# ssteinberg/wave_tracer

Measured on AMD Instinct MI355X. Metric: Msamples/sec (whole node), cornell-box 1440^2 wave-mode, higher is better.
Workload: dtype f32

## Files before the change

### wave_tracer_amd/api.py

```python
import ctypes as C
import json
import math
import os

_HERE = os.path.dirname(os.path.abspath(__file__))

os.environ.setdefault("HSA_KERNARG_POOL_SIZE", str(16 << 20))


def lib_path():
    return os.environ.get("WTGPU_LIB") or os.path.join(_HERE, "libwtgpu.so")


class WtgpuError(RuntimeError):
    pass


class SceneParams(C.Structure):
    _fields_ = [("res", C.c_uint32), ("max_depth", C.c_int32), ("fsd", C.c_int32), ("mis", C.c_int32), ("rr", C.c_int32),
                ("force_ray_tracing", C.c_int32), ("mesh_detail", C.c_int32), ("lut_n_theta", C.c_uint32), ("lut_m", C.c_uint32),
                ("polarimetric", C.c_int32)]


class TestHooks(C.Structure):
# ... 65 lines not shown


SYMBOLS = ["wtgpu_scene_create_named", "wtgpu_scene_create_from_desc", "wtgpu_scene_get_info", "wtgpu_scene_host_desc",
           "wtgpu_scene_upload", "wtgpu_render", "wtgpu_trace_rays", "wtgpu_traverse_cones", "wtgpu_get_counters",
           "wtgpu_reset_counters", "wtgpu_last_render_timings", "wtgpu_develop", "wtgpu_scene_destroy", "wtgpu_last_error",
           "wtgpu_scene_stats_json", "wtgpu_calibrate_copy", "wtgpu_render_async", "wtgpu_join", "wtgpu_query_regions", "wtgpu_render_progressive",
           "wtgpu_cancel", "wtgpu_pause", "wtgpu_resume", "wtgpu_capture_intermediate", "wtgpu_comm_unique_id", "wtgpu_comm_create", "wtgpu_film_reduce", "wtgpu_comm_destroy", "wtgpu_scene_create_from_xml",
           "wtgpu_scene_shape_id", "wtgpu_scene_sensor_mask_spec", "wtgpu_sensor_mask", "wtgpu_sensor_mask_host",
           "wtgpu_scene_tonemap_spec", "wtgpu_develop_device", "wtgpu_tonemap_device", "wtgpu_tonemap_host",
           "wtgpu_film_stats_edges", "wtgpu_film_stats_device", "wtgpu_film_stats_host",
           "wtgpu_film_compare_device", "wtgpu_film_compare_host"]
PROGRESS_CB = C.CFUNCTYPE(C.c_int, C.c_uint64, C.c_uint64, C.c_void_p)
CAPTURE_CB = C.CFUNCTYPE(None, C.c_uint64, C.c_void_p)

_lib = None


def load_library():
    global _lib
    if _lib is not None:
        return _lib
    p = lib_path()
    if not os.path.exists(p):
        raise WtgpuError(f"{p} is missing: build it with `python -c 'import __graft_entry__ as g; g.build()'` "
                         f"(hipcc --offload-arch=gfx950); wave_tracer_amd has no CPU fallback")
    os.environ.setdefault("HSA_KERNARG_POOL_SIZE", str(16 << 20))
    try:
        import torch
    except ImportError:
        pass
# ... 541 lines not shown
        def call(spec, rec, planes):
            if diff:
                d["diff"] = np.zeros((self.height, self.width, planes), dtype=np.float32)
            _check(load_library().wtgpu_film_compare_host(self._h, *(t.ctypes.data for t in sets[0]), int(spe_a), *(t.ctypes.data for t in sets[1]), int(spe_b),
                                                          C.byref(spec), None if m is None else m.ctypes.data, int(threads), C.cast(rec, C.c_void_p),
                                                          d["diff"].ctypes.data if diff else None))
        out = self._film_compare(call, stokes_component, abs, luminance, eps)
        out.update(d)
        return out

    def profile_counters(self, n=8):
        out = (C.c_uint64 * n)()
        _check(load_library().wtgpu_test_profile_counters(self._h, out, n))
        return [int(v) for v in out]

    def counters(self):
        c = Counters()
        _check(load_library().wtgpu_get_counters(self._h, C.byref(c)))
        return c.as_dict()

    def reset_counters(self):
        _check(load_library().wtgpu_reset_counters(self._h))

    def trace_ab_stats(self):
        a, b, d, w, r = C.c_double(0), C.c_double(0), C.c_uint64(0), C.c_uint64(0), C.c_uint64(0)
        _check(load_library().wtgpu_trace_ab_stats(self._h, C.byref(a), C.byref(b), C.byref(d), C.byref(w), C.byref(r)))
        return {"ms_refill": a.value, "ms_sm": b.value, "differing_words": int(d.value), "walks": int(w.value), "rounds": int(r.value)}

    def timings(self):
        t = (C.c_float * 12)()
# ... 46 lines not shown
```

### wave_tracer_amd/csrc/kernels_connect.hip

```cpp
#include "wtgpu_kernels.h"

namespace wtk {

WT_D bool strategy_valid(const integrator_opts_t& o, int s, int t, int nS, int nT) {
    const int depth = t + s - 2;
    if (t > nT || s > nS) return false;
    if ((t == 1 && s == 1) || depth < 0 || depth > o.max_depth) return false;
    if (!o.emitter_direct && s == 1) return false;
    if (!o.sensor_direct && t == 1) return false;
    if (o.debug_only_s && (int)o.debug_only_s - 1 != s) return false;
    if (o.debug_only_t && (int)o.debug_only_t - 1 != t) return false;
    return true;
}
WT_D bool strategy_class_valid(const integrator_opts_t& o, int sk, int tk, int nS, int nT) {
    const int K = (int)kKeyDim - 1;
    const int t1 = tk < K ? tk : nT, s1 = sk < K ? sk : nS;
    for (int t = tk; t <= t1; ++t)
        for (int s = sk; s <= s1; ++s)
            if (strategy_valid(o, s, t, nS, nT)) return true;
    return false;
}
WT_D int wave_max_i(int v) {
#pragma unroll
    for (int off = 32; off > 0; off >>= 1) v = max(v, __shfl_xor(v, off, 64));
    return v;
}

__global__ void __launch_bounds__(kEnumBlock) k_connect_enum(launch_args_t a) {
    __shared__ uint32_t s_cnt[kNumKeys], s_base[kNumKeys];
    const uint32_t i = blockIdx.x * kEnumBlock + threadIdx.x;
    const size_t W2 = 2 * (size_t)a.st.cap;
    for (uint32_t k = threadIdx.x; k < kNumKeys; k += kEnumBlock) s_cnt[k] = 0;
    int nT = -1, nS = -1;
    if (i < a.nb) {
        nT = (int)a.st.walks[(size_t)(i) * a.st.walk_words + WT_WALK_NVERTS_WORD];
        nS = (int)a.st.walks[(size_t)(a.st.cap + i) * a.st.walk_words + WT_WALK_NVERTS_WORD];
#pragma unroll
        for (int c = 0; c < 4; ++c) a.st.lacc[(size_t)c * a.st.cap + i] = 0.0;
    }
    __syncthreads();
    const int K = (int)kKeyDim - 1;
    const int kT = nT < K ? nT : K, kS = nS < K ? nS : K;
    for (int tk = 0; tk <= kT; ++tk)
        for (int sk = 0; sk <= kS; ++sk)
            if (strategy_class_valid(a.sc.opts, sk, tk, nS, nT)) atomicAdd(&s_cnt[(uint32_t)tk * kKeyDim + (uint32_t)sk], 1u);
    __syncthreads();
    for (uint32_t k = threadIdx.x; k < kNumKeys; k += kEnumBlock) {
        const uint32_t c = s_cnt[k];
        s_base[k] = c ? atomicAdd(a.st.strat_count + k, c) : 0u;
        s_cnt[k] = 0;
    }
    __syncthreads();
    for (int tk = 0; tk <= kT; ++tk)
        for (int sk = 0; sk <= kS; ++sk)
            if (strategy_class_valid(a.sc.opts, sk, tk, nS, nT)) {
                const uint32_t key = (uint32_t)tk * kKeyDim + (uint32_t)sk;
                a.st.strat_items[(size_t)key * a.st.cap + s_base[key] + atomicAdd(&s_cnt[key], 1u)] = i;
            }
}
__global__ void __launch_bounds__(64) k_connect_scan(launch_args_t a) {
    if (a.st.ext)
        for (uint32_t q = threadIdx.x; q < a.st.ext->n_chunks * kChunkCtlWords; q += 64) a.st.ext->chunk_ctl[q] = 0;
    if (threadIdx.x == 0) {
        uint32_t acc = 0;
        for (uint32_t k = 0; k < kNumKeys; ++k) {
            const uint32_t c = a.st.strat_count[k];
            a.st.strat_prefix[k] = acc;
            acc += c;
            a.st.strat_count[k] = 0;
        }
        a.st.strat_prefix[kNumKeys] = acc;
        a.st.ctl[CTL_STRAT_HEAD] = 0;
        a.st.ctl[CTL_STRAT_HEAD_OPEN] = 0;

    }
}
template <bool OPEN>
WT_D void connect_strat_body(const launch_args_t& a) {
    __shared__ stack_entry_t lds[kLdsStack * kBlock];
    __shared__ uint32_t s_prefix[kNumKeys + 1];
    constexpr int K = (int)kKeyDim - 1;
    if (!OPEN) {
        for (uint32_t k = threadIdx.x; k <= kNumKeys; k += kBlock) s_prefix[k] = a.st.strat_prefix[k];
    } else if (threadIdx.x == 0) {
        uint32_t acc = 0;
        for (uint32_t k = 0; k < kNumKeys; ++k) {
            s_prefix[k] = acc;
            if ((int)(k / kKeyDim) == K || (int)(k % kKeyDim) == K) acc += a.st.strat_prefix[k + 1] - a.st.strat_prefix[k];
        }
// ... 42 lines not shown
                one(sk, tk);
            } else {
                const int nT = (int)a.st.walks[(size_t)i * a.st.walk_words + WT_WALK_NVERTS_WORD];
                const int nS = (int)a.st.walks[((size_t)a.st.cap + i) * a.st.walk_words + WT_WALK_NVERTS_WORD];
                const int t1 = tk == K ? nT : tk, s1 = sk == K ? nS : sk;
                for (int t = tk; t <= t1; ++t)
                    for (int s = sk; s <= s1; ++s)
                        if (strategy_valid(a.sc.opts, s, t, nS, nT)) one(s, t);
            }
        }
    }
    if (a.count_stats) flush_counters(a.st.counters, ctr);
}
__global__ void __launch_bounds__(kBlock, WTGPU_LB_CONNECT) k_connect_strat(launch_args_t a) { connect_strat_body<false>(a); }
__global__ void __launch_bounds__(kBlock, WTGPU_LB_CONNECT) k_connect_strat_open(launch_args_t a) { connect_strat_body<true>(a); }
constexpr uint32_t kPendShadow = 0x80000000u;
WT_D void pending_append(const launch_args_t& a, uint32_t* cctl, bool keep, uint32_t i, int s, int t, const connect_ret_t& cr) {
    const bdpt_ext_t& x = *a.st.ext;
    const unsigned long long m = __ballot(keep);
    if (!m) return;
    const int lane = threadIdx.x & 63;
    const int leader = __ffsll((long long)m) - 1;
    uint32_t base = 0;
    if (lane == leader) base = atomicAdd(cctl + CHUNK_PEND_COUNT, (uint32_t)__popcll(m));
    base = (uint32_t)__shfl((int)base, leader, 64);
    const uint32_t slot = base + (uint32_t)__popcll(m & ((1ull << lane) - 1ull));
    if (!keep || slot >= x.pend_cap) return;
    conn_pending_t r;
    r.i = i;
    r.st = (uint32_t)s | ((uint32_t)t << 16) | (cr.need_shadow ? kPendShadow : 0u);
// ... 215 lines not shown
```

### wave_tracer_amd/csrc/wtgpu.hip

```cpp
#include "wtgpu_host.h"

thread_local std::string g_err;

static void note_rounds(wtgpu_scene* s, uint32_t n) { s->rounds_hist[s->rounds_hist_n++ % 8u] = n; }
static int drain_rec(wtgpu_scene* s, chunk_rec_t& r) {
    if (!r.busy) return WTGPU_OK;
    HIP_CHECK(hipEventSynchronize(r.ev[r.ev_final]));
    const uint32_t rounds = r.h_ctl[CTL_ROUNDS];
    s->cap_hits += r.h_ctl[CTL_COUNT0 + (r.rounds_launched & 1u)] + r.h_ctl[CTL_BACK0 + (r.rounds_launched & 1u)];
    s->acc[4] += rounds;
    s->acc[5] += rounds;
    s->acc[6] += 1;
    s->rounds_launched_total += r.rounds_launched;
    if (s->knobs.timing) {
        auto elapsed = [](hipEvent_t a, hipEvent_t b) {
            float ms = 0.f;
            return hipEventElapsedTime(&ms, a, b) == hipSuccess ? ms : 0.f;
        };
        s->acc[0] += elapsed(r.ev[0], r.ev[1]);
        size_t e = 1;
        for (uint32_t k = 0; k < r.rounds_timed; ++k, e += 6) {
            static const int slot[6] = {1, 7, 2, 8, 9, 10};
            for (int q = 0; q < 6; ++q) s->acc[slot[q]] += elapsed(r.ev[e + q], r.ev[e + q + 1]);
        }
// ... 144 lines not shown
            HP_LAUNCH(k_interact_c_hard, dim3(std::max<uint32_t>(1u, gh / K.grid_div_hard)), dim3(WTGPU_HARD_BLOCK), 0, st_, a, in);
            rec(r, st_);
        }
        r.rounds_launched = r_end;
        return WTGPU_OK;
    }
    void light(const launch_args_t& a, hipStream_t st_, uint32_t launched) {
        if (path_mode || !K.light_rounds || launched >= K.max_rounds) return;
        HP_LAUNCH(k_light_rounds, dim3(1), dim3(kBlock), 0, st_, a, (int)(launched & 1u), launched, K.max_rounds - launched);
    }
    int tail(const launch_args_t& a, chunk_rec_t& r, hipStream_t st_) {
        const uint32_t nb = a.nb, gf = g_full(nb);
        if (path_mode) {
            HP_LAUNCH(k_path_flush, dim3(kFlushGrid), dim3(kBlock), 0, st_, a, (int)(r.rounds_launched & 1u));
        } else {
            HP_LAUNCH(k_connect_enum, dim3((nb + kEnumBlock - 1) / kEnumBlock), dim3(kEnumBlock), 0, st_, a);
            HP_LAUNCH(k_connect_scan, dim3(1), dim3(64), 0, st_, a);
            const bool open = (uint32_t)s->host.opts.max_depth + 2 >= kKeyDim - 1;
            if (K.staged_connect && !open) {
                for (uint32_t c = 0; c < s->n_chunks; ++c) {
                    const uint32_t g = c == 0 ? gf : std::max<uint32_t>(1u, gf / 8u);
                    HP_LAUNCH(k_connect_eval, dim3(g), dim3(kBlock), 0, st_, a, c);
                    HP_LAUNCH(k_connect_shadow, dim3(g), dim3(kBlock), 0, st_, a, c);
                    HP_LAUNCH(k_connect_mis, dim3(g), dim3(kBlock), 0, st_, a, c);
                }
            } else {
                HP_LAUNCH(k_connect_strat, dim3(gf), dim3(kBlock), 0, st_, a);
                if (open) HP_LAUNCH(k_connect_strat_open, dim3(std::max<uint32_t>(1u, gf / 8u)), dim3(kBlock), 0, st_, a);
            }
            const uint32_t fw = a.film.width, fh = a.film.height, planes = film_planes(s->host.sensor);
            if (K.tiled_splat && s->host.sensor.rf_radius <= 1 && planes <= 16 && (uint64_t)nb * 2u >= (uint64_t)a.npix)
                HP_LAUNCH(k_connect_splat_tiled, dim3(fh * ((fw + kBlock - 1) / kBlock)), dim3(kBlock), 3 * kSplatCols * (planes + 1) * sizeof(double), st_, a);
            else
                HP_LAUNCH(k_connect_splat, dim3((nb + kBlock - 1) / kBlock), dim3(kBlock), 0, st_, a);
        }
        HIP_CHECK(hipGetLastError());
        HIP_CHECK(hipMemcpyAsync(r.h_ctl, a.st.ctl, CTL_WORDS * sizeof(uint32_t), hipMemcpyDeviceToHost, st_));
        r.ev_final = s->knobs.timing ? r.ev_used : 0;
        HIP_CHECK(hipEventRecord(r.ev[r.ev_final], st_));
        if (ev_fail) return fail(WTGPU_ERR_HIP, "hipEventRecord failed");
// ... 229 lines not shown
```

### wave_tracer_amd/csrc/wtgpu_kernels.h

```cpp
#pragma once
#include <hip/hip_runtime.h>

#include <cstddef>
#include <cstdint>
#include <cstring>

#include "../../include/wtgpu.h"
#include "wt/bdpt.h"
#include "wt/coop.h"
#include "wt/coop_fsd.h"
#include "wt/coop_utd.h"
#include "wt/path.h"

using namespace wt;
namespace wt {
struct tonemap_args_t;
}

namespace wtk {


#ifndef WTGPU_LB_TRACE
#define WTGPU_LB_TRACE 3
#endif
// ... 23 lines not shown
constexpr int kLdsStack = WTGPU_LDS_STACK;
constexpr uint32_t kConeBudget = 96;
constexpr int kSpillStack = 64 - kLdsStack;

enum : uint32_t { CTL_STRAT_HEAD_OPEN = 25, CTL_UTD_COUNT0 = 26, CTL_UTD_COUNT1 = 27, CTL_FSDQ_COUNT0 = 28, CTL_FSDQ_COUNT1 = 29, CTL_FSDQ_HEAD = 30, CTL_NEEQ_COUNT = 31, CTL_NEEQ_HEAD = 32, CTL_COUNT0 = 0, CTL_COUNT1 = 1, CTL_HEAD_TRACE = 2, CTL_HEAD_INTERACT = 3, CTL_HEAVY_COUNT = 4, CTL_HEAVY_HEAD = 5, CTL_FSD_COUNTER = 6,
                  CTL_ROUNDS = 7, CTL_STRAT_HEAD = 8, CTL_INTB_COUNT = 9, CTL_INTB_HEAD = 10, CTL_GATHER_COUNT = 11, CTL_GATHER_HEAD = 12, CTL_INTC_COUNT = 13, CTL_INTC_HEAD = 14, CTL_FTASK_COUNT = 15, CTL_FTASK_HEAD = 16, CTL_FSPLIT_HEAD = 17, CTL_EPOOL_COUNT = 18, CTL_FSD_ECOUNTER = 19, CTL_INTD_COUNT = 20, CTL_INTD_HEAD = 21, CTL_BACK0 = 22, CTL_BACK1 = 23,
                  CTL_TPOL_COUNT0 = 41, CTL_TPOL_COUNT1 = 42, CTL_TPOL_HEAD = 43, CTL_TCONE_COUNT0 = 44, CTL_TCONE_COUNT1 = 45, CTL_TCONE_HEAD = 46,
                  CTL_CLS_COUNT0 = 33, CTL_CLS_HEAD0 = 37,
                  CTL_LIGHT_DONE = 47, CTL_LIGHT_STOP = 48,
                  CTL_WORDS = 56 };
constexpr uint32_t kTriListWords = 128;
constexpr uint32_t kGatherMarker = 0xFFFFFFFEu;
constexpr uint32_t kApertureMarker = 0xFFFFFFFDu, kNullApertureMarker = 0xFFFFFFFCu;
__host__ __device__ inline bool is_region_marker(uint32_t t) { return t == kGatherMarker || t == kApertureMarker; }
constexpr uint32_t kKeyDim = kMaxVerts + 2, kNumKeys = kKeyDim * kKeyDim;

struct device_state_t {
    uint64_t cap = 0;
    uint32_t max_verts = 0;
    uint32_t walk_words = 0;
    size_t vert_words = 0;
    uint32_t* walks = nullptr;
    uint32_t* verts = nullptr;
    uint32_t* ctx = nullptr;
    uint32_t* trav = nullptr;
    uint32_t* tris = nullptr;
    uint32_t* queue[2] = {nullptr, nullptr};
    uint32_t* heavy_queue = nullptr;
    uint32_t* intb_queue = nullptr;
    uint32_t* gather_queue = nullptr;
// ... 226 lines not shown
__global__ void k_interact_coop(launch_args_t a, int in, int first_round);
__global__ void k_edges(launch_args_t a);
__global__ void k_interact_b(launch_args_t a, int in);
__global__ void k_light_rounds(launch_args_t a, int in, uint32_t round, uint32_t max_rounds);
__global__ void k_flux_split(launch_args_t a);
__global__ void k_flux_tasks(launch_args_t a);
__global__ void k_interact_c(launch_args_t a, int in);
__global__ void k_interact_c_hard(launch_args_t a, int in);
__global__ void k_path_generate(launch_args_t a);
__global__ void k_path_fsd(launch_args_t a, const path_state_t* __restrict__ ps, uint32_t round);
__global__ void k_path_edges(launch_args_t a, const path_state_t* __restrict__ ps);
__global__ void k_path_interact(launch_args_t a, const path_state_t* __restrict__ ps, int in, int first_round, uint32_t round);
__global__ void k_path_interact_b(launch_args_t a, const path_state_t* __restrict__ ps, int in, uint32_t round);
__global__ void k_path_nee(launch_args_t a, const path_state_t* __restrict__ ps, uint32_t round);
__global__ void k_path_flush(launch_args_t a, int in);
__global__ void k_connect_enum(launch_args_t a);
__global__ void k_connect_scan(launch_args_t a);
__global__ void k_connect_strat(launch_args_t a);
__global__ void k_connect_strat_open(launch_args_t a);
__global__ void k_connect_eval(launch_args_t a, uint32_t chunk);
__global__ void k_connect_shadow(launch_args_t a, uint32_t chunk);
__global__ void k_connect_mis(launch_args_t a, uint32_t chunk);
__global__ void k_connect_splat(launch_args_t a);
__global__ void k_connect_splat_tiled(launch_args_t a);
__global__ void k_calib_copy(const uint32_t* in, uint32_t* out, size_t n);
__global__ void k_trace_rays(scene_t sc, const float* rays, uint32_t n, float* dist, uint32_t* tuid, float* bary, uint32_t* front);
__global__ void k_traverse_cones(scene_t sc, const float* cones, uint32_t n, uint32_t cap, float* dist, uint32_t* flags, uint32_t* ntris, uint32_t* out_tris,
                                 uint32_t* scratch_tris);
__global__ void k_query_regions(scene_t sc, const float* cones, uint32_t n, uint32_t edge_cap, float* dist, uint32_t* flags, uint32_t* primary, uint32_t* ntris,
                                uint32_t* nedges, uint32_t* edges, float* flux, unsigned long long* dropped);
int test_fsd_apertures(const scene_t& sc, hipStream_t stream, const float* d_cones, const float* d_sk, const uint32_t* d_ids, const uint32_t* d_n_ids,
                       uint32_t n, uint32_t id_cap, uint32_t pool_cap, uint32_t mode, uint32_t* d_hdr, float* d_segs);
int test_utd_sums(const scene_t& sc, hipStream_t stream, const float* d_queries, const uint32_t* d_ids, const uint32_t* d_n_ids, uint32_t n, uint32_t id_cap,
                  uint32_t utd_cap, uint32_t* d_recs, uint32_t* d_hdr, uint32_t* d_edges);
// ... 26 lines not shown
```

### wave_tracer_amd/csrc/wtgpu_knobs.h

```cpp
#pragma once
#include <cstddef>
#include <cstdint>

struct knobs_t {
    uint32_t cone_budget, count_stats, split_queues, lane_cache, heavy_cache, heavy_probe, coop_aperture_min, flux_task_tris, profile, no_lists, primary_axis;
    uint32_t streams, state_gb, timing, conn_pool;
    uint32_t first_rounds, rounds_margin, light_rounds, max_rounds, stagger_round;
    uint32_t shrink_r1, shrink_f1, shrink_r2, shrink_f2, shrink_h1, decay_q, decay_c;
    uint32_t heavy_waves_per_cu, round_blocks_per_cu, grid_div_b, grid_div_c, grid_div_hard, grid_mul_flux;
    uint32_t sorted_interact, coop_io, staged_connect, tiled_splat;
    uint32_t trace_staged, trace_stages, trace_staged_rounds, trace_sm, trace_ab;
    uint32_t develop_per_pixel, tonemap_lds_table;
    uint32_t dbg_stage;
    uint32_t host_prof, trace_launch, tail_diag, trace_ab_verbose;
    uint32_t grid_div_cls[4];
};

enum knob_kind_t {
    KNOB_U32,
    KNOB_INT,
    KNOB_NONZERO,
    KNOB_PRESENT
};
struct knob_t {
    const char* name;
// ... 13 lines not shown
```

### wave_tracer_amd/csrc/wtgpu_knobs.hip

```cpp
#include "wtgpu_knobs.h"

#include <algorithm>
#include <climits>
#include <cstdio>
#include <cstdlib>

#include "wt/bdpt.h"

using wt::kMaxWalkIters;
using wt::kWalkIterLimit;

#define K(field) &knobs_t::field
static constexpr long long kU32 = 0xFFFFFFFFll;
const knob_t kKnobs[] = {
    {"WTGPU_CONE_BUDGET", K(cone_budget), KNOB_U32, kKnobConeBudget, 0, kU32, "work units one lane may spend on a cone query before it is handed to a wavefront (wtgpu_kernels.h: kConeBudget)"},
    {"WTGPU_COUNT_STATS", K(count_stats), KNOB_U32, 1, 0, kU32, "0: the kernels keep no statistics (wtgpu_kernels.h: launch_args_t::count_stats)"},
    {"WTGPU_SPLIT_QUEUES", K(split_queues), KNOB_U32, 1, 0, kU32, "round queues keep sensor and emitter walks apart; 0: one mixed queue (A/B)"},
    {"WTGPU_LANE_CACHE", K(lane_cache), KNOB_U32, 1, 0, kU32, "0 (diagnostic): the per-lane traversal without its remembered rejecting triangles"},
    {"WTGPU_HEAVY_CACHE", K(heavy_cache), KNOB_U32, 1, 0, kU32, "0 (diagnostic): the wave-cooperative traversal without its remembered rejecting triangles"},
    {"WTGPU_HEAVY_PROBE", K(heavy_probe), KNOB_U32, 1, 0, kU32, "k_trace_heavy: any-hit probe of the near slab before the handed-over cone query too; 0: off"},
    {"WTGPU_COOP_APERTURE_MIN", K(coop_aperture_min), KNOB_U32, 8, 0, kU32, "segments from which an aperture is built by a wavefront; 0xFFFFFFFF: every aperture by a single lane of pass B"},
    {"WTGPU_FLUX_TASK_TRIS", K(flux_task_tris), KNOB_U32, kKnobFluxTaskTris, 64, kU32, "triangles per region-sum task (k_flux_split / k_flux_tasks; wtgpu_kernels.h: kFluxTaskTris)"},
    {"WTGPU_PROFILE", K(profile), KNOB_U32, 0, 0, kU32, "1 / 2 / 3: in-kernel clock breakdowns, printed by wtgpu_get_counters (wtgpu_counters.hip)"},
    {"WTGPU_NO_LISTS", K(no_lists), KNOB_PRESENT, 0, 0, 1, "set (any value; plt_bdpt, diagnostic): no bounded triangle lists, every interaction region is gathered"},
// ... 11 lines not shown
    {"WTGPU_SHRINK_F1", K(shrink_f1), KNOB_U32, 4, 1, kU32, "see WTGPU_SHRINK_R1"},
    {"WTGPU_SHRINK_R2", K(shrink_r2), KNOB_U32, 16, 0, kU32, "from this round on the grids are divided by WTGPU_SHRINK_F2 (heavy: 32)"},
    {"WTGPU_SHRINK_F2", K(shrink_f2), KNOB_U32, 32, 1, kU32, "see WTGPU_SHRINK_R2"},
    {"WTGPU_SHRINK_H1", K(shrink_h1), KNOB_U32, 4, 1, kU32, "see WTGPU_SHRINK_R1"},
    {"WTGPU_DECAY_Q", K(decay_q), KNOB_U32, 0, 0, kU32, "per cent; > 0: grids follow WTGPU_DECAY_C x q^round instead of the step schedule above"},
    {"WTGPU_DECAY_C", K(decay_c), KNOB_U32, 4, 1, kU32, "safety factor of the geometric schedule"},
    {"WTGPU_HEAVY_WAVES", K(heavy_waves_per_cu), KNOB_U32, 8, 1, kU32, "wavefronts per CU of the wave-per-item kernels; swept 6 / 8 / 10 / 12 / 16 / 24 / 32: 169.6 / 168.0 / 171.6 / 174.3 / 176 / 181 / 183 ms per pass"},
    {"WTGPU_ROUND_BLOCKS", K(round_blocks_per_cu), KNOB_U32, 8, 1, kU32, "blocks per CU of the round kernels' persistent grids"},
    {"WTGPU_GRID_B", K(grid_div_b), KNOB_U32, 4, 1, kU32, "pass B's grid relative to the round's (divisor)"},
    {"WTGPU_GRID_C", K(grid_div_c), KNOB_U32, 1, 1, kU32, "pass C's grid (divisor); 2 until round 4; 1: bidir_room 33.6 -> 33.9, cornell 25.15 -> 25.35 Msamples/s, pass C's bracket 69 -> 56 / 93 -> 65 ms"},
    {"WTGPU_GRID_HARD", K(grid_div_hard), KNOB_U32, 4, 1, kU32, "k_interact_c_hard's grid (divisor)"},
    {"WTGPU_GRID_FLUX", K(grid_mul_flux), KNOB_U32, 2, 1, kU32, "k_flux_tasks' grid (multiplier)"},
    {"WTGPU_SORTED_INTERACT", K(sorted_interact), KNOB_U32, 0, 0, kU32, "pass A: 0 k_interact (one kernel, every walk); 1 k_classify + one kernel per material class; 2 k_classify + k_interact_sorted"},
    {"WTGPU_COOP_IO", K(coop_io), KNOB_U32, 0, 0, kU32, "1: pass A with wave-cooperative record transfers (k_interact_coop)"},
    {"WTGPU_STAGED_CONNECT", K(staged_connect), KNOB_U32, 0, 0, kU32, "connections: 0 k_connect_strat (one kernel per strategy item); 1 k_connect_eval -> k_connect_shadow -> k_connect_mis, in chunks"},
    {"WTGPU_TILED_SPLAT", K(tiled_splat), KNOB_U32, 1, 0, kU32, "0: the plain per-sample splat kernel"},
    {"WTGPU_TRACE_STAGED", K(trace_staged), KNOB_U32, 1, 0, kU32, "1: the traversal in stages (k_tr_axis / k_tr_cone / k_tr_policy / k_tr_tail) ..."},
    {"WTGPU_TRACE_STAGES", K(trace_stages), KNOB_U32, 3, 1, 16, "... with this many cone stages before the tail ..."},
    {"WTGPU_TRACE_STAGED_ROUNDS", K(trace_staged_rounds), KNOB_U32, 4, 0, kU32, "... for the first so many rounds of a batch (the long ones: a stage is a launch, and a short round is bound by its launches)"},
    {"WTGPU_TRACE_SM", K(trace_sm), KNOB_U32, 0, 0, kU32, "1: the phase-machine trace kernel (k_trace_sm)"},
    {"WTGPU_TRACE_AB", K(trace_ab), KNOB_U32, 0, 0, kU32, "n: the first n rounds replay their trace queue through both trace kernels, timed, outputs compared (wtgpu_trace_ab.hip)"},
    {"WTGPU_DEVELOP_PER_PIXEL", K(develop_per_pixel), KNOB_U32, 0, 0, 1, "k_develop: 0 one lane per plane element; 1 one lane per pixel (A/B: tools/bench_develop.py)"},
    {"WTGPU_TONEMAP_LDS_TABLE", K(tonemap_lds_table), KNOB_U32, 0, 0, 1, "k_develop_tonemap: 1 every block stages the colour table in LDS; 0 the lanes read it through the caches (A/B: tools/bench_develop.py)"},
    {"WTGPU_DEBUG_STAGE", K(dbg_stage), KNOB_INT, 1 << 30, INT_MIN, INT_MAX, "bring-up aid: stops launching the round kernels after stage n (INVALID RESULTS)"},
    {"WTGPU_HOST_PROF", K(host_prof), KNOB_PRESENT, 0, 0, 1, "set: host time spent inside each kind of launch call, printed per render call"},
    {"WTGPU_TRACE_LAUNCH", K(trace_launch), KNOB_PRESENT, 0, 0, 1, "set (bring-up aid): every launch is named and waited for — the last line names a kernel that hangs"},
    {"WTGPU_TAIL_DIAG", K(tail_diag), KNOB_PRESENT, 0, 0, 1, "set: why the host was called back for a pending batch, printed at exit (DESIGN.md §9)"},
    {"WTGPU_TRACE_AB_VERBOSE", K(trace_ab_verbose), KNOB_PRESENT, 0, 0, 1, "set: one line per round replayed by WTGPU_TRACE_AB"},
};
#undef K
// ... 18 lines not shown
```

### wave_tracer_amd/csrc/wtgpu_queries.hip

```cpp
#include "wtgpu_host.h"
#include "wt/sources_probe.h"

extern "C" {

int wtgpu_trace_rays(wtgpu_scene* s, void* stream_, const float* d_rays, uint32_t n, float* d_dist, uint32_t* d_tuid, float* d_bary, uint32_t* d_front) {
    if (!s || !s->uploaded) return fail(WTGPU_ERR_INVALID, "scene not uploaded");
    hipStream_t stream = static_cast<hipStream_t>(stream_);
    hipLaunchKernelGGL(k_trace_rays, dim3((n + kBlock - 1) / kBlock), dim3(kBlock), 0, stream, s->dev, d_rays, n, d_dist, d_tuid, d_bary, d_front);
    HIP_CHECK(hipGetLastError());
    return WTGPU_OK;
}
int wtgpu_traverse_cones(wtgpu_scene* s, void* stream_, const float* d_cones, uint32_t n, uint32_t cap, float* d_dist, uint32_t* d_flags,
                         uint32_t* d_ntris, uint32_t* d_tris) {
    if (!s || !s->uploaded) return fail(WTGPU_ERR_INVALID, "scene not uploaded");
    hipStream_t stream = static_cast<hipStream_t>(stream_);
    const size_t need = (size_t)n * kMaxConeTris * 4 * 2;
    if (need > s->query_scratch_bytes) {
        device_guard_t guard(s->device);
        void* p = nullptr;
        HIP_CHECK(hipMalloc(&p, need));
        s->dev_allocs.push_back(p);
        s->query_scratch = static_cast<uint32_t*>(p);
        s->query_scratch_bytes = need;
    }
// ... 97 lines not shown
    if (!s || !s->uploaded) return fail(WTGPU_ERR_INVALID, "scene not uploaded");
    if (n == 0) return WTGPU_OK;
    if (!d_queries || !d_out) return fail(WTGPU_ERR_INVALID, "null argument");
    hipStream_t stream = static_cast<hipStream_t>(stream_);
    device_guard_t guard(s->device);
    std::vector<uint32_t> q((size_t)n * kSourceProbeQueryWords);
    HIP_CHECK(hipMemcpyAsync(q.data(), d_queries, q.size() * sizeof(uint32_t), hipMemcpyDeviceToHost, stream));
    HIP_CHECK(hipStreamSynchronize(stream));
    for (uint32_t i = 0; i < n; ++i)
        if (!source_probe_query_ok(s->host, q.data() + (size_t)i * kSourceProbeQueryWords))
            return fail(WTGPU_ERR_INVALID, "wtgpu_test_source_queries: query " + std::to_string(i) + ": op, emitter index or tuid out of range");
    HIP_CHECK((hipError_t)test_source_queries(s->dev, stream, d_queries, n, d_out));
    return WTGPU_OK;
}

int wtgpu_calibrate_copy(uint64_t n_dwords, int repeats) {
    uint32_t *in = nullptr, *out = nullptr;
    HIP_CHECK(hipMalloc((void**)&in, n_dwords * 4));
    HIP_CHECK(hipMalloc((void**)&out, n_dwords * 4));
    HIP_CHECK(hipMemset(in, 1, n_dwords * 4));
    for (int r = 0; r < repeats; ++r) hipLaunchKernelGGL(k_calib_copy, dim3(256 * 32), dim3(256), 0, 0, in, out, (size_t)n_dwords);
    HIP_CHECK(hipDeviceSynchronize());
    HIP_CHECK(hipFree(in));
    HIP_CHECK(hipFree(out));
    return WTGPU_OK;
}

}
```

### wave_tracer_amd/csrc/wtgpu_test_hooks.h

```cpp
#pragma once
#include "../../include/wtgpu.h"
#ifdef __cplusplus
extern "C" {
#endif
typedef struct wtgpu_test_hooks {
    uint32_t only_s, only_t;
    uint32_t crop_of;
} wtgpu_test_hooks;
int wtgpu_scene_create_named_hooks(const char* name, const wtgpu_scene_params* params, const wtgpu_test_hooks* hooks, wtgpu_scene** out);
int wtgpu_scene_compare(const wtgpu_scene* a, const wtgpu_scene* b, char* what, size_t n_what);
int wtgpu_scene_compare_part(const wtgpu_scene* a, const wtgpu_scene* b, const char* part, char* what, size_t n_what);
int wtgpu_trace_ab_stats(wtgpu_scene* s, double* ms_refill, double* ms_sm, uint64_t* differing_words, uint64_t* walks, uint64_t* rounds);
int wtgpu_test_profile_counters(wtgpu_scene* s, unsigned long long* out, uint32_t n);
int wtgpu_test_fsd_apertures(wtgpu_scene* s, void* stream, const float* d_cones, const float* d_sk, const uint32_t* d_ids, const uint32_t* d_n_ids,
                             uint32_t n, uint32_t id_cap, uint32_t pool_cap, uint32_t mode, uint32_t* d_hdr, float* d_segs);
int wtgpu_test_utd_sums(wtgpu_scene* s, void* stream, const float* d_queries, const uint32_t* d_ids, const uint32_t* d_n_ids, uint32_t n, uint32_t id_cap,
                        uint32_t utd_cap, uint32_t* d_recs, uint32_t* d_hdr, uint32_t* d_edges);
int wtgpu_test_bsdf_queries(wtgpu_scene* s, void* stream, const uint32_t* d_queries, uint32_t n, int form, uint32_t* d_out);
int wtgpu_test_source_queries(wtgpu_scene* s, void* stream, const uint32_t* d_queries, uint32_t n, uint32_t* d_out);
#ifdef __cplusplus
}
#endif
```

### wave_tracer_amd/csrc/wtgpu_upload.hip

```cpp
#include "wtgpu_host.h"

static int g_env_by_host = 0;
__attribute__((constructor)) static void wtgpu_runtime_settings() {
    if (getenv("HSA_KERNARG_POOL_SIZE")) g_env_by_host |= 1;
    setenv("HSA_KERNARG_POOL_SIZE", "16777216", 0);
}
static int runtime_settings_ok(std::string& why) {
    const char* k = getenv("HSA_KERNARG_POOL_SIZE");
    const long ring = k ? atol(k) : (1l << 20);
    if (getenv("WTGPU_ALLOW_SLOW_RUNTIME")) return 1;
    if (ring < (4l << 20)) {
        why = "HSA_KERNARG_POOL_SIZE=" + std::string(k ? k : "(unset)") + ": a batch enqueues ~900 launches of ~1 KB of kernel arguments; with a ring below 4 MiB the enqueueing "
              "thread blocks and the streams serialise; export HSA_KERNARG_POOL_SIZE=16777216 before the HIP runtime initialises, or WTGPU_ALLOW_SLOW_RUNTIME=1";
        return 0;
    }
    if (!(g_env_by_host & 1) && !getenv("WTGPU_QUIET")) {
        static bool told = false;
        if (!told) fprintf(stderr, "[wtgpu] note: HSA_KERNARG_POOL_SIZE=16777216 defaulted by libwtgpu.so; effective only if the HIP runtime had not initialised before the library was loaded "
                           "(a host that uses HIP earlier exports it itself, INTEGRATION.md)\n");
        told = true;
    }
    return 1;
}

// ... 146 lines not shown
    if ((rc = dmalloc(s, &st.intc_queue, W2))) return rc;
    if ((rc = dmalloc(s, &st.intd_queue, W2))) return rc;
    st.ftask_cap = path_mode ? 1u : (1u << 22);
    if ((rc = dmalloc(s, &st.ftasks, (size_t)st.ftask_cap))) return rc;
    if ((rc = dmalloc(s, &st.facc, path_mode ? 1 : W2))) return rc;
    st.epool_cap = 1u << 23;
    if ((rc = dmalloc(s, &st.epool, (size_t)st.epool_cap))) return rc;
    if ((rc = dmalloc(s, &st.ctl, (size_t)CTL_WORDS))) return rc;
    HIP_CHECK(hipMemset(st.ctl, 0, CTL_WORDS * sizeof(uint32_t)));
    st.fsd_cap = (h.opts.FSD && !h.opts.force_ray_tracing && !path_mode) ? (uint32_t)std::min<uint64_t>(W2, 1u << 22) : 1u;
    if ((rc = dmalloc(s, &st.fsd_hdr, st.fsd_cap))) return rc;
    st.fsd_ecap = st.fsd_cap > 1 ? (uint32_t)std::min<uint64_t>(64ull * st.cap + kFsdMaxEdges, 1ull << 28) : 1u;
    if ((rc = dmalloc(s, &st.fsd_edges, (size_t)st.fsd_ecap))) return rc;
    if ((rc = dmalloc(s, &st.strat_items, path_mode ? 1 : (size_t)kNumKeys * st.cap))) return rc;
    if ((rc = dmalloc(s, &st.strat_count, (size_t)kNumKeys))) return rc;
    if ((rc = dmalloc(s, &st.strat_prefix, (size_t)kNumKeys + 1))) return rc;
    if ((rc = dmalloc(s, &st.lacc, 4 * (size_t)st.cap))) return rc;
    HIP_CHECK(hipMemset(st.strat_count, 0, kNumKeys * sizeof(uint32_t)));
    HIP_CHECK(hipStreamCreateWithFlags(&s->streams[k], hipStreamNonBlocking));
    HIP_CHECK(hipEventCreateWithFlags(&s->ev_done[k], hipEventDisableTiming));
    return WTGPU_OK;
}

static uint64_t size_batches(const wtgpu_scene* s, uint64_t max_batch, uint32_t& n_slices) {
    const scene_t& h = s->host;
    const uint64_t npix = (uint64_t)h.sensor.width * h.sensor.height;
    n_slices = s->knobs.streams;
    uint64_t batch_cap = max_batch ? std::min<uint64_t>(max_batch, 1u << 24) : std::min<uint64_t>(npix, 1u << 22);
    n_slices = (uint32_t)std::min<uint64_t>(n_slices, std::max<uint64_t>(1, batch_cap / 64));
    {
        const bool pm = h.opts.integrator != INTEGRATOR_BDPT;
// ... 115 lines not shown
```

Before: 32.07.

## Bucket BDPT connections per sample by subpath-length class, evaluating all strategies in-thread

Adds a connection mode, on by default, where each sample is enqueued once under a key set by its camera and light subpath lengths. Classes are ordered by descending work and padded to wave multiples, so a wave gets samples of equal shape and runs every strategy in a row, summing flux locally. This removes the per-strategy item expansion and lacc accumulation, and is meant to reduce divergence and atomics. In exchange each item is much longer and per-thread work is less balanced, and test hooks are added to read the class table.

```diff
diff --git a/wave_tracer_amd/api.py b/wave_tracer_amd/api.py
--- a/wave_tracer_amd/api.py
+++ b/wave_tracer_amd/api.py
@@ -103,6 +103,17 @@
 CAPTURE_CB = C.CFUNCTYPE(None, C.c_uint64, C.c_void_p)
 
 _lib = None
+
+
+def connect_class_order():
+    import numpy as np
+    lib = load_library()
+    lib.wtgpu_test_connect_class_order.argtypes = [C.c_void_p, C.c_uint32, C.c_void_p, C.c_void_p]
+    n, dim = C.c_uint32(0), C.c_uint32(0)
+    _check(lib.wtgpu_test_connect_class_order(None, 0, C.byref(n), C.byref(dim)))
+    keys = np.zeros(n.value, np.uint32)
+    _check(lib.wtgpu_test_connect_class_order(keys.ctypes.data, keys.size, C.byref(n), C.byref(dim)))
+    return keys, int(dim.value)
 
 
 def load_library():
@@ -674,6 +685,17 @@
         _check(load_library().wtgpu_test_profile_counters(self._h, out, n))
         return [int(v) for v in out]
 
+    def connect_class_items(self, slice=0, max_items=1 << 22):
+        import numpy as np
+        lib = load_library()
+        lib.wtgpu_test_connect_class_items.argtypes = [C.c_void_p, C.c_uint32, C.c_void_p, C.c_void_p, C.c_uint32, C.c_void_p]
+        n_keys = connect_class_order()[0].size
+        table = np.zeros(3 * n_keys + 1, np.uint32)
+        items = np.zeros(max_items, np.uint32)
+        n = C.c_uint32(0)
+        _check(lib.wtgpu_test_connect_class_items(self._h, slice, table.ctypes.data, items.ctypes.data, items.size, C.byref(n)))
+        return table[:n_keys + 1].copy(), table[n_keys + 1:2 * n_keys + 1].copy(), table[2 * n_keys + 1:].copy(), items[:n.value].copy()
+
     def counters(self):
         c = Counters()
         _check(load_library().wtgpu_get_counters(self._h, C.byref(c)))
diff --git a/wave_tracer_amd/csrc/kernels_connect.hip b/wave_tracer_amd/csrc/kernels_connect.hip
--- a/wave_tracer_amd/csrc/kernels_connect.hip
+++ b/wave_tracer_amd/csrc/kernels_connect.hip
@@ -26,21 +26,35 @@
     return v;
 }
 
-__global__ void __launch_bounds__(kEnumBlock) k_connect_enum(launch_args_t a) {
+__global__ void __launch_bounds__(kEnumBlock) k_connect_enum(launch_args_t a, uint32_t by_class) {
     __shared__ uint32_t s_cnt[kNumKeys], s_base[kNumKeys];
     const uint32_t i = blockIdx.x * kEnumBlock + threadIdx.x;
-    const size_t W2 = 2 * (size_t)a.st.cap;
     for (uint32_t k = threadIdx.x; k < kNumKeys; k += kEnumBlock) s_cnt[k] = 0;
     int nT = -1, nS = -1;
     if (i < a.nb) {
         nT = (int)a.st.walks[(size_t)(i) * a.st.walk_words + WT_WALK_NVERTS_WORD];
         nS = (int)a.st.walks[(size_t)(a.st.cap + i) * a.st.walk_words + WT_WALK_NVERTS_WORD];
-#pragma unroll
-        for (int c = 0; c < 4; ++c) a.st.lacc[(size_t)c * a.st.cap + i] = 0.0;
+        if (!by_class) {
+#pragma unroll
+            for (int c = 0; c < 4; ++c) a.st.lacc[(size_t)c * a.st.cap + i] = 0.0;
+        }
     }
     __syncthreads();
     const int K = (int)kKeyDim - 1;
     const int kT = nT < K ? nT : K, kS = nS < K ? nS : K;
+    if (by_class) {
+        const uint32_t key = (uint32_t)max(kT, 0) * kKeyDim + (uint32_t)max(kS, 0);
+        if (i < a.nb) atomicAdd(&s_cnt[key], 1u);
+        __syncthreads();
+        for (uint32_t k = threadIdx.x; k < kNumKeys; k += kEnumBlock) {
+            const uint32_t c = s_cnt[k];
+            s_base[k] = c ? atomicAdd(a.st.strat_count + k, c) : 0u;
+            s_cnt[k] = 0;
+        }
+        __syncthreads();
+        if (i < a.nb) a.st.strat_items[(size_t)key * a.st.cap + s_base[key] + atomicAdd(&s_cnt[key], 1u)] = i;
+        return;
+    }
     for (int tk = 0; tk <= kT; ++tk)
         for (int sk = 0; sk <= kS; ++sk)
             if (strategy_class_valid(a.sc.opts, sk, tk, nS, nT)) atomicAdd(&s_cnt[(uint32_t)tk * kKeyDim + (uint32_t)sk], 1u);
@@ -58,21 +72,30 @@
                 a.st.strat_items[(size_t)key * a.st.cap + s_base[key] + atomicAdd(&s_cnt[key], 1u)] = i;
             }
 }
-__global__ void __launch_bounds__(64) k_connect_scan(launch_args_t a) {
+__global__ void __launch_bounds__(64) k_connect_scan(launch_args_t a, uint32_t by_class) {
+    __shared__ uint32_t s_key[kNumKeys];
     if (a.st.ext)
         for (uint32_t q = threadIdx.x; q < a.st.ext->n_chunks * kChunkCtlWords; q += 64) a.st.ext->chunk_ctl[q] = 0;
+    if (by_class)
+        for (uint32_t k = threadIdx.x; k < kNumKeys; k += 64) s_key[class_key_rank(k)] = k;
+    __syncthreads();
     if (threadIdx.x == 0) {
         uint32_t acc = 0;
-        for (uint32_t k = 0; k < kNumKeys; ++k) {
+        for (uint32_t r = 0; r < kNumKeys; ++r) {
+            const uint32_t k = by_class ? s_key[r] : r;
             const uint32_t c = a.st.strat_count[k];
-            a.st.strat_prefix[k] = acc;
-            acc += c;
+            a.st.strat_prefix[r] = acc;
+            if (by_class) {
+                a.st.strat_prefix[kClassCount + r] = c;
+                a.st.strat_prefix[kClassKey + r] = k;
+                acc += (c + 63u) & ~63u;
+            } else
+                acc += c;
             a.st.strat_count[k] = 0;
         }
         a.st.strat_prefix[kNumKeys] = acc;
         a.st.ctl[CTL_STRAT_HEAD] = 0;
         a.st.ctl[CTL_STRAT_HEAD_OPEN] = 0;
-
     }
 }
 template <bool OPEN>
@@ -145,6 +168,80 @@
 }
 __global__ void __launch_bounds__(kBlock, WTGPU_LB_CONNECT) k_connect_strat(launch_args_t a) { connect_strat_body<false>(a); }
 __global__ void __launch_bounds__(kBlock, WTGPU_LB_CONNECT) k_connect_strat_open(launch_args_t a) { connect_strat_body<true>(a); }
+template <bool OPEN>
+WT_D void connect_class_body(const launch_args_t& a) {
+    __shared__ stack_entry_t lds[kLdsStack * kBlock];
+    __shared__ uint32_t s_prefix[kNumKeys + 1], s_count[kNumKeys], s_key[kNumKeys];
+    constexpr int K = (int)kKeyDim - 1;
+    for (uint32_t r = threadIdx.x; r < kNumKeys; r += kBlock) {
+        s_count[r] = a.st.strat_prefix[kClassCount + r];
+        s_key[r] = a.st.strat_prefix[kClassKey + r];
+    }
+    if (!OPEN) {
+        for (uint32_t r = threadIdx.x; r <= kNumKeys; r += kBlock) s_prefix[r] = a.st.strat_prefix[r];
+    } else if (threadIdx.x == 0) {
+        uint32_t acc = 0;
+        for (uint32_t r = 0; r < kNumKeys; ++r) {
+            s_prefix[r] = acc;
+            if (class_key_open(a.st.strat_prefix[kClassKey + r])) acc += (a.st.strat_prefix[kClassCount + r] + 63u) & ~63u;
+        }
+        s_prefix[kNumKeys] = acc;
+    }
+    __syncthreads();
+    const uint32_t total = s_prefix[kNumKeys];
+    const uint32_t lane = threadIdx.x & 63;
+    bdpt_counters_t ctr;
+    memset(&ctr, 0, sizeof(ctr));
+    stack_entry_t spill[kSpillStack];
+    stack_ref_t stack;
+    lds_stack(lds, spill, stack);
+    const fsd_pool_t pool{a.st.fsd_hdr, a.st.fsd_edges, a.st.ctl + CTL_FSD_COUNTER, a.st.fsd_cap, a.st.ctl + CTL_FSD_ECOUNTER, a.st.fsd_ecap};
+    for (;;) {
+        const uint32_t base = wave_grab(a.st.ctl + (OPEN ? CTL_STRAT_HEAD_OPEN : CTL_STRAT_HEAD));
+        if (base >= total) break;
+        uint32_t lo = 0, hi = kNumKeys;
+        while (hi - lo > 1) {
+            const uint32_t mid = (lo + hi) >> 1;
+            if (s_prefix[mid] <= base)
+                lo = mid;
+            else
+                hi = mid;
+        }
+        const uint32_t rank = uniform(lo), key = uniform(s_key[rank]);
+        const int tk = (int)(key / kKeyDim), sk = (int)(key % kKeyDim);
+        const uint32_t off = base - uniform(s_prefix[rank]) + lane;
+        if (class_key_open(key) == OPEN && off < uniform(s_count[rank])) {
+            const uint32_t i = a.st.strat_items[(size_t)key * a.st.cap + off];
+            const uint64_t j = a.j0 + i;
+            const uint32_t pix = (uint32_t)(j % a.npix);
+            const uint64_t smp = a.sample_begin + j / a.npix;
+            const uint64_t sample_id = ((uint64_t)pix << 32) | (smp & 0xFFFFFFFFull);
+            sample_ctx_t ctx;
+            soa_load(a.st.ctx, kCtxWords, i, ctx);
+            const vertex_store_t svs{a.st.verts, a.st.vert_words, i}, evs{a.st.verts, a.st.vert_words, (size_t)a.st.cap + i};
+            int nT = tk, nS = sk;
+            if constexpr (OPEN) {
+                nT = (int)a.st.walks[(size_t)i * a.st.walk_words + WT_WALK_NVERTS_WORD];
+                nS = (int)a.st.walks[((size_t)a.st.cap + i) * a.st.walk_words + WT_WALK_NVERTS_WORD];
+            }
+            double sum[4] = {0.0, 0.0, 0.0, 0.0};
+            for (int t = 0; t <= nT; ++t)
+                for (int s = 0; s <= nS; ++s)
+                    if (strategy_valid(a.sc.opts, s, t, nS, nT)) {
+                        const stokes_t flux = bdpt_strategy(a.sc, pool, a.film, svs, evs, s, t, ctx, a.seed, sample_id, stack, &ctr, nullptr);
+                        if (t > 1) {
+#pragma unroll
+                            for (int c = 0; c < 4; ++c) sum[c] += (double)flux.s[c];
+                        }
+                    }
+#pragma unroll
+            for (int c = 0; c < 4; ++c) a.st.lacc[(size_t)c * a.st.cap + i] = sum[c];
+        }
+    }
+    if (a.count_stats) flush_counters(a.st.counters, ctr);
+}
+__global__ void __launch_bounds__(kBlock, WTGPU_LB_CONNECT) k_connect_class(launch_args_t a) { connect_class_body<false>(a); }
+__global__ void __launch_bounds__(kBlock, WTGPU_LB_CONNECT) k_connect_class_open(launch_args_t a) { connect_class_body<true>(a); }
 constexpr uint32_t kPendShadow = 0x80000000u;
 WT_D void pending_append(const launch_args_t& a, uint32_t* cctl, bool keep, uint32_t i, int s, int t, const connect_ret_t& cr) {
     const bdpt_ext_t& x = *a.st.ext;
diff --git a/wave_tracer_amd/csrc/wtgpu.hip b/wave_tracer_amd/csrc/wtgpu.hip
--- a/wave_tracer_amd/csrc/wtgpu.hip
+++ b/wave_tracer_amd/csrc/wtgpu.hip
@@ -182,16 +182,21 @@
         if (path_mode) {
             HP_LAUNCH(k_path_flush, dim3(kFlushGrid), dim3(kBlock), 0, st_, a, (int)(r.rounds_launched & 1u));
         } else {
-            HP_LAUNCH(k_connect_enum, dim3((nb + kEnumBlock - 1) / kEnumBlock), dim3(kEnumBlock), 0, st_, a);
-            HP_LAUNCH(k_connect_scan, dim3(1), dim3(64), 0, st_, a);
             const bool open = (uint32_t)s->host.opts.max_depth + 2 >= kKeyDim - 1;
-            if (K.staged_connect && !open) {
+            const bool staged = K.staged_connect && !open;
+            const uint32_t by_class = !staged && K.connect_class ? 1u : 0u;
+            HP_LAUNCH(k_connect_enum, dim3((nb + kEnumBlock - 1) / kEnumBlock), dim3(kEnumBlock), 0, st_, a, by_class);
+            HP_LAUNCH(k_connect_scan, dim3(1), dim3(64), 0, st_, a, by_class);
+            if (staged) {
                 for (uint32_t c = 0; c < s->n_chunks; ++c) {
                     const uint32_t g = c == 0 ? gf : std::max<uint32_t>(1u, gf / 8u);
                     HP_LAUNCH(k_connect_eval, dim3(g), dim3(kBlock), 0, st_, a, c);
                     HP_LAUNCH(k_connect_shadow, dim3(g), dim3(kBlock), 0, st_, a, c);
                     HP_LAUNCH(k_connect_mis, dim3(g), dim3(kBlock), 0, st_, a, c);
                 }
+            } else if (by_class) {
+                HP_LAUNCH(k_connect_class, dim3(gf), dim3(kBlock), 0, st_, a);
+                if (open) HP_LAUNCH(k_connect_class_open, dim3(std::max<uint32_t>(1u, gf / 8u)), dim3(kBlock), 0, st_, a);
             } else {
                 HP_LAUNCH(k_connect_strat, dim3(gf), dim3(kBlock), 0, st_, a);
                 if (open) HP_LAUNCH(k_connect_strat_open, dim3(std::max<uint32_t>(1u, gf / 8u)), dim3(kBlock), 0, st_, a);
diff --git a/wave_tracer_amd/csrc/wtgpu_kernels.h b/wave_tracer_amd/csrc/wtgpu_kernels.h
--- a/wave_tracer_amd/csrc/wtgpu_kernels.h
+++ b/wave_tracer_amd/csrc/wtgpu_kernels.h
@@ -61,6 +61,15 @@
 constexpr uint32_t kApertureMarker = 0xFFFFFFFDu, kNullApertureMarker = 0xFFFFFFFCu;
 __host__ __device__ inline bool is_region_marker(uint32_t t) { return t == kGatherMarker || t == kApertureMarker; }
 constexpr uint32_t kKeyDim = kMaxVerts + 2, kNumKeys = kKeyDim * kKeyDim;
+__host__ __device__ constexpr uint32_t class_key_work(uint32_t key) { return (key / kKeyDim) * (key % kKeyDim); }
+__host__ __device__ constexpr uint32_t class_key_rank(uint32_t key) {
+    uint32_t r = 0;
+    for (uint32_t k = 0; k < kNumKeys; ++k)
+        if (class_key_work(k) > class_key_work(key) || (class_key_work(k) == class_key_work(key) && k < key)) ++r;
+    return r;
+}
+__host__ __device__ constexpr bool class_key_open(uint32_t key) { return key / kKeyDim == kKeyDim - 1 || key % kKeyDim == kKeyDim - 1; }
+constexpr uint32_t kClassCount = kNumKeys + 1, kClassKey = kClassCount + kNumKeys, kClassTableWords = kClassKey + kNumKeys;
 
 struct device_state_t {
     uint64_t cap = 0;
@@ -317,10 +326,12 @@
 __global__ void k_path_interact_b(launch_args_t a, const path_state_t* __restrict__ ps, int in, uint32_t round);
 __global__ void k_path_nee(launch_args_t a, const path_state_t* __restrict__ ps, uint32_t round);
 __global__ void k_path_flush(launch_args_t a, int in);
-__global__ void k_connect_enum(launch_args_t a);
-__global__ void k_connect_scan(launch_args_t a);
+__global__ void k_connect_enum(launch_args_t a, uint32_t by_class);
+__global__ void k_connect_scan(launch_args_t a, uint32_t by_class);
 __global__ void k_connect_strat(launch_args_t a);
 __global__ void k_connect_strat_open(launch_args_t a);
+__global__ void k_connect_class(launch_args_t a);
+__global__ void k_connect_class_open(launch_args_t a);
 __global__ void k_connect_eval(launch_args_t a, uint32_t chunk);
 __global__ void k_connect_shadow(launch_args_t a, uint32_t chunk);
 __global__ void k_connect_mis(launch_args_t a, uint32_t chunk);
diff --git a/wave_tracer_amd/csrc/wtgpu_knobs.h b/wave_tracer_amd/csrc/wtgpu_knobs.h
--- a/wave_tracer_amd/csrc/wtgpu_knobs.h
+++ b/wave_tracer_amd/csrc/wtgpu_knobs.h
@@ -8,7 +8,7 @@
     uint32_t first_rounds, rounds_margin, light_rounds, max_rounds, stagger_round;
     uint32_t shrink_r1, shrink_f1, shrink_r2, shrink_f2, shrink_h1, decay_q, decay_c;
     uint32_t heavy_waves_per_cu, round_blocks_per_cu, grid_div_b, grid_div_c, grid_div_hard, grid_mul_flux;
-    uint32_t sorted_interact, coop_io, staged_connect, tiled_splat;
+    uint32_t sorted_interact, coop_io, staged_connect, connect_class, tiled_splat;
     uint32_t trace_staged, trace_stages, trace_staged_rounds, trace_sm, trace_ab;
     uint32_t develop_per_pixel, tonemap_lds_table;
     uint32_t dbg_stage;
diff --git a/wave_tracer_amd/csrc/wtgpu_knobs.hip b/wave_tracer_amd/csrc/wtgpu_knobs.hip
--- a/wave_tracer_amd/csrc/wtgpu_knobs.hip
+++ b/wave_tracer_amd/csrc/wtgpu_knobs.hip
@@ -49,6 +49,7 @@
     {"WTGPU_SORTED_INTERACT", K(sorted_interact), KNOB_U32, 0, 0, kU32, "pass A: 0 k_interact (one kernel, every walk); 1 k_classify + one kernel per material class; 2 k_classify + k_interact_sorted"},
     {"WTGPU_COOP_IO", K(coop_io), KNOB_U32, 0, 0, kU32, "1: pass A with wave-cooperative record transfers (k_interact_coop)"},
     {"WTGPU_STAGED_CONNECT", K(staged_connect), KNOB_U32, 0, 0, kU32, "connections: 0 k_connect_strat (one kernel per strategy item); 1 k_connect_eval -> k_connect_shadow -> k_connect_mis, in chunks"},
+    {"WTGPU_CONNECT_CLASS", K(connect_class), KNOB_U32, 1, 0, kU32, "connections (the one-kernel form): 0 k_connect_strat (an item is one strategy of a sample); 1 k_connect_class (an item is a sample, bucketed by the lengths of its subpaths, all of its strategies in a row; DESIGN.md §4)"},
     {"WTGPU_TILED_SPLAT", K(tiled_splat), KNOB_U32, 1, 0, kU32, "0: the plain per-sample splat kernel"},
     {"WTGPU_TRACE_STAGED", K(trace_staged), KNOB_U32, 1, 0, kU32, "1: the traversal in stages (k_tr_axis / k_tr_cone / k_tr_policy / k_tr_tail) ..."},
     {"WTGPU_TRACE_STAGES", K(trace_stages), KNOB_U32, 3, 1, 16, "... with this many cone stages before the tail ..."},
diff --git a/wave_tracer_amd/csrc/wtgpu_queries.hip b/wave_tracer_amd/csrc/wtgpu_queries.hip
--- a/wave_tracer_amd/csrc/wtgpu_queries.hip
+++ b/wave_tracer_amd/csrc/wtgpu_queries.hip
@@ -135,6 +135,41 @@
     return WTGPU_OK;
 }
 
+int wtgpu_test_connect_class_order(uint32_t* keys, uint32_t cap, uint32_t* n_keys, uint32_t* key_dim) {
+    if (!n_keys || !key_dim) return fail(WTGPU_ERR_INVALID, "wtgpu_test_connect_class_order: null argument");
+    *n_keys = kNumKeys;
+    *key_dim = kKeyDim;
+    if (!keys || cap < kNumKeys) return WTGPU_OK;
+    for (uint32_t r = 0; r < kNumKeys; ++r) keys[r] = 0xFFFFFFFFu;
+    for (uint32_t k = 0; k < kNumKeys; ++k) {
+        const uint32_t r = class_key_rank(k);
+        if (r < kNumKeys) keys[r] = k;
+    }
+    return WTGPU_OK;
+}
+
+int wtgpu_test_connect_class_items(wtgpu_scene* s, uint32_t slice, uint32_t* table, uint32_t* items, uint32_t items_cap, uint32_t* n_items) {
+    if (!s || !s->uploaded || !table || !items || !n_items || slice >= s->slices.size()) return fail(WTGPU_ERR_INVALID, "wtgpu_test_connect_class_items: uploaded scene, a slice of it");
+    if (s->host.opts.integrator != INTEGRATOR_BDPT) return fail(WTGPU_ERR_INVALID, "wtgpu_test_connect_class_items: plt_bdpt scenes");
+    device_guard_t guard(s->device);
+    {
+        const int rc = drain_all(s);
+        if (rc) return rc;
+    }
+    HIP_CHECK(hipDeviceSynchronize());
+    const device_state_t& st = s->slices[slice];
+    HIP_CHECK(hipMemcpy(table, st.strat_prefix, kClassTableWords * sizeof(uint32_t), hipMemcpyDeviceToHost));
+    uint64_t n = 0;
+    for (uint32_t r = 0; r < kNumKeys; ++r) {
+        const uint32_t c = table[kClassCount + r], key = table[kClassKey + r];
+        if (key >= kNumKeys || c > st.cap || n + c > items_cap) return fail(WTGPU_ERR_INVALID, "wtgpu_test_connect_class_items: not a class table (was the batch connected by k_connect_class?) or items_cap too small");
+        if (c) HIP_CHECK(hipMemcpy(items + n, st.strat_items + (size_t)key * st.cap, c * sizeof(uint32_t), hipMemcpyDeviceToHost));
+        n += c;
+    }
+    *n_items = (uint32_t)n;
+    return WTGPU_OK;
+}
+
 int wtgpu_calibrate_copy(uint64_t n_dwords, int repeats) {
     uint32_t *in = nullptr, *out = nullptr;
     HIP_CHECK(hipMalloc((void**)&in, n_dwords * 4));
diff --git a/wave_tracer_amd/csrc/wtgpu_test_hooks.h b/wave_tracer_amd/csrc/wtgpu_test_hooks.h
--- a/wave_tracer_amd/csrc/wtgpu_test_hooks.h
+++ b/wave_tracer_amd/csrc/wtgpu_test_hooks.h
@@ -18,6 +18,8 @@
                         uint32_t utd_cap, uint32_t* d_recs, uint32_t* d_hdr, uint32_t* d_edges);
 int wtgpu_test_bsdf_queries(wtgpu_scene* s, void* stream, const uint32_t* d_queries, uint32_t n, int form, uint32_t* d_out);
 int wtgpu_test_source_queries(wtgpu_scene* s, void* stream, const uint32_t* d_queries, uint32_t n, uint32_t* d_out);
+int wtgpu_test_connect_class_order(uint32_t* keys, uint32_t cap, uint32_t* n_keys, uint32_t* key_dim);
+int wtgpu_test_connect_class_items(wtgpu_scene* s, uint32_t slice, uint32_t* table, uint32_t* items, uint32_t items_cap, uint32_t* n_items);
 #ifdef __cplusplus
 }
 #endif
diff --git a/wave_tracer_amd/csrc/wtgpu_upload.hip b/wave_tracer_amd/csrc/wtgpu_upload.hip
--- a/wave_tracer_amd/csrc/wtgpu_upload.hip
+++ b/wave_tracer_amd/csrc/wtgpu_upload.hip
@@ -184,7 +184,7 @@
     if ((rc = dmalloc(s, &st.fsd_edges, (size_t)st.fsd_ecap))) return rc;
     if ((rc = dmalloc(s, &st.strat_items, path_mode ? 1 : (size_t)kNumKeys * st.cap))) return rc;
     if ((rc = dmalloc(s, &st.strat_count, (size_t)kNumKeys))) return rc;
-    if ((rc = dmalloc(s, &st.strat_prefix, (size_t)kNumKeys + 1))) return rc;
+    if ((rc = dmalloc(s, &st.strat_prefix, (size_t)kClassTableWords))) return rc;
     if ((rc = dmalloc(s, &st.lacc, 4 * (size_t)st.cap))) return rc;
     HIP_CHECK(hipMemset(st.strat_count, 0, kNumKeys * sizeof(uint32_t)));
     HIP_CHECK(hipStreamCreateWithFlags(&s->streams[k], hipStreamNonBlocking));
```

After: 32.57, median of 6. 1.02x the previous value.
